# ext-sakamoro/ALICE-Codec

Measured on AMD Instinct MI355X. Metric: Mpixels/s encode+decode, 1080p x 64 CDF9/7 q=80; bit-exact vs CPU, higher is better.
Workload: dtype int32

## Files before the change

alice-codec_amd/csrc/codec.hip:

```cpp
#include <hip/hip_runtime.h>
#include <sys/mman.h>

#include <algorithm>
#include <atomic>
#include <chrono>
#include <condition_variable>
#include <cmath>
#include <cstdio>
#include <cstdlib>
#include <cstring>
#include <exception>
#include <map>
#include <memory>
#include <mutex>
#include <new>
#include <string>
#include <thread>
#include <vector>

#include "../../include/alice_codec.h"
#include "../../include/alice_codec_test.h"
#include "common.h"
#include "kernels.h"

// ... 859 lines not shown
                                 w.hist.as<uint32_t>() + (size_t)b * 3 * 256, w.results.as<RansResult>() + 3 * b,
                                 w.sizes.as<unsigned long long>() + b, 1, st);
    launch_compact_streams(w.alc.as<uint8_t>(), w.alc_stride, kStreamHead, w.cap, w.results.as<RansResult>(), B, st);
    if (evs) HIP_TRY(hipEventRecord(evs->ev[4], st));
    HIP_TRY(hipGetLastError());
    return kOk;
}

int encode_flags_error(uint32_t flags) {
    if (flags & kTableDiverges)
        return fail(kReferenceDiverges, "a symbol whose table frequency wrapped to 0 is present: the reference encoder does not terminate on this input");
    if (flags & kRansInternal) return fail(kInternal, "rANS kernel invariant violated");
    return kOk;
}

constexpr int kOverflowed = -1;

int encode_collect(EncodeWork& w, hipStream_t st, std::vector<RansResult>& res) {
    res.resize((size_t)w.n_chunks * 3);
    HIP_TRY(hipMemcpyAsync(res.data(), w.results.p, res.size() * sizeof(RansResult), hipMemcpyDeviceToHost, st));
    HIP_TRY(hipStreamSynchronize(st));
    for (auto& r : res) TRY(encode_flags_error(r.flags));
    if (debug_on())
        for (size_t i = 0; i < res.size(); ++i)
            fprintf(stderr, "[alice] encode chain %zu: %llu bytes, %.1f Mcycles, %.1f ms of 100 MHz ticks => %.2f GHz, xcc %u se %u cu %u simd %u\n", i, res[i].len,
                    res[i].cycles_k * 1024.0 / 1e6, res[i].ticks_k * 1024.0 / 1e5,
                    res[i].ticks_k ? (res[i].cycles_k / (double)res[i].ticks_k) * 0.1 : 0.0,
                    res[i].xcc_id & 15u, (res[i].hw_id >> 13) & 7u, (res[i].hw_id >> 8) & 15u, (res[i].hw_id >> 4) & 3u);
    for (auto& r : res)
        if (r.flags & kRansOverflow) return kOverflowed;
    return kOk;
}

int encode_with_retry(const RgbLayout* rgb, EncodeWork& w, uint8_t quality, int wavelet, hipStream_t st, StageEvents* evs,
                      CapMode mode, HubTicket* hub, std::vector<RansResult>& res, const uint8_t* qualities = nullptr) {
    for (int m = mode; m <= kCapWorst; ++m) {
        TRY(encode_launch(rgb, w, quality, wavelet, st, evs, (CapMode)m, hub, qualities));
        const int rc = encode_collect(w, st, res);
        if (rc != kOverflowed) return rc;
    }
    return fail(kInternal, "rANS output exceeded the worst-case capacity");
}

struct DecodeWork {
    ChunkDims d{};
    int n_chunks = 0;
    DevBuf scratch_own, gen, tmp, sym, hist, tables, descs, results, planes;
    uint8_t* sym_ptr = nullptr;
    DevBuf* scratch = nullptr;
};

int decode_work_alloc(DecodeWork& w, const ChunkDims& d, int n_chunks, uint8_t* sym_ext = nullptr, DevBuf* scratch_ext = nullptr) {
    w.d = d; w.n_chunks = n_chunks;
    w.scratch = scratch_ext ? scratch_ext : &w.scratch_own;
    if (sym_ext) w.sym_ptr = sym_ext;
    else { TRY(w.sym.alloc((size_t)n_chunks * 3 * d.padded)); w.sym_ptr = w.sym.as<uint8_t>(); }
    TRY(w.hist.alloc((size_t)n_chunks * 3 * 256 * sizeof(uint32_t)));
    TRY(w.tables.alloc((size_t)n_chunks * 3 * sizeof(RansTable)));
    TRY(w.descs.alloc((size_t)n_chunks * 3 * sizeof(RansDecodeDesc)));
    TRY(w.results.alloc((size_t)n_chunks * 3 * sizeof(RansResult)));
    return kOk;
}

int inverse_chunk(const uint8_t* d_sym, const ChunkDims& d, int wavelet, const int32_t step[3], void* d_scratch, DecodeWork& w,
                  const RgbLayout& rgb, hipStream_t st, SplitFormat fmt = kFormatSplit) {
    const bool wide = is_wide(fmt), mirror = fmt == kFormatReversible;
    const InverseBounds ib = inverse_bounds(wavelet, step, wide ? kWideMaxQ : kByteMaxQ);
    if (mirror) {
        if (d_scratch && launch_inverse_transform_reversible((const uint16_t*)d_sym, d, wavelet, step, ib.exact, ib.mid16, ib.lds16, d_scratch, rgb, st))
            return kOk;
    } else if (wide) {
        if (d_scratch && launch_inverse_transform_wide((const uint16_t*)d_sym, d, wavelet, step, ib.exact, ib.mid16, ib.lds16, d_scratch, rgb, st))
            return kOk;
    } else if (d_scratch && launch_inverse_transform(d_sym, d, wavelet, step, ib.exact, ib.mid16, ib.lds16, d_scratch, rgb, st)) return kOk;
    if (!w.planes.p) TRY(w.planes.alloc(3 * d.n_pixels * sizeof(int16_t)));
    if (!w.tmp.p) TRY(w.tmp.alloc(d.padded * sizeof(int32_t)));
    if (!w.gen.p) TRY(w.gen.alloc(2 * d.padded * sizeof(int32_t)));
    int16_t* pl = w.planes.as<int16_t>();
    int32_t* qb = w.gen.as<int32_t>();
    int32_t* vol = qb + d.padded;
    const uint64_t W = d.pw, H = d.ph, D = d.pf;
    for (int c = 0; c < 3; ++c) {
        if (wide) launch_from_symbols_wide((const uint16_t*)d_sym + (size_t)c * d.padded, qb, d.padded, st);
        else launch_from_symbols(d_sym + (size_t)c * d.padded, qb, d.padded, st);
        launch_dequantize(qb, vol, d.padded, step[c], st);
        launch_wavelet_axis(vol, w.tmp.as<int32_t>(), D, W * H, 1, 0, W * H, 1, wavelet, true, st, mirror);
        launch_wavelet_axis(vol, w.tmp.as<int32_t>(), H, W, D, W * H, W, 1, wavelet, true, st, mirror);
        launch_wavelet_axis(vol, w.tmp.as<int32_t>(), W, 1, D * H, W, 1, 0, wavelet, true, st, mirror);
        launch_strip_channel(vol, d, pl + (size_t)c * d.n_pixels, st);
    }
    launch_ycocg_to_rgb(pl, pl + d.n_pixels, pl + 2 * d.n_pixels, d, rgb, st);
    return kOk;
}

int decode_launch(const EncodedChunk* const* headers, const std::vector<const uint8_t*>& d_payload,
                  DecodeWork& w, const std::vector<RgbLayout>& rgb, hipStream_t st, StageEvents* evs, HubTicket* hub = nullptr) {
    const ChunkDims& d = w.d;
    const int B = w.n_chunks;
    if (transform_tiles_eligible(d)) {
        bool all16 = true;
        for (int b = 0; b < B; ++b) {
            const int32_t step[3] = {headers[b]->ch[0].quant_step, headers[b]->ch[1].quant_step, headers[b]->ch[2].quant_step};
            all16 = all16 && inverse_bounds(headers[b]->wavelet, step).mid16;
        }
        const size_t need = inverse_scratch_bytes(d, all16);
        if (!w.scratch->p || w.scratch->n < need) {
            HIP_TRY(hipStreamSynchronize(st));
            TRY(w.scratch->alloc(need));
        }
    }
    std::vector<uint32_t> hist((size_t)B * 3 * 256);
    std::vector<RansDecodeDesc> descs((size_t)B * 3);
    for (int b = 0; b < B; ++b) {
        uint64_t off = 0;
        for (int c = 0; c < 3; ++c) {
            const ChannelHeader& h = headers[b]->ch[c];
            memcpy(&hist[((size_t)b * 3 + c) * 256], h.histogram, 256 * sizeof(uint32_t));
            RansDecodeDesc& ds = descs[(size_t)b * 3 + c];
            ds.in = d_payload[b] + off;
            ds.in_len = h.compressed_len;
            ds.out = w.sym_ptr + ((size_t)b * 3 + c) * d.padded;
            ds.n = d.padded;
            ds.table = w.tables.as<RansTable>() + ((size_t)b * 3 + c);
            off += h.compressed_len;
        }
    }
    HIP_TRY(hipMemcpyAsync(w.hist.p, hist.data(), hist.size() * sizeof(uint32_t), hipMemcpyHostToDevice, st));
    if (!hub) HIP_TRY(hipMemcpyAsync(w.descs.p, descs.data(), descs.size() * sizeof(RansDecodeDesc), hipMemcpyHostToDevice, st));
    HIP_TRY(hipStreamSynchronize(st));
    if (evs) HIP_TRY(hipEventRecord(evs->ev[5], st));
    launch_rans_table(w.hist.as<uint32_t>(), w.tables.as<RansTable>(), 3 * B, st);
    if (hub) {
        for (size_t c = 0; c < descs.size(); ++c) descs[c].result = w.results.as<RansResult>() + c;
        TRY(hub_chains(st, {}, std::move(descs), d.padded, hub));
    } else {
        launch_rans_decode(w.descs.as<RansDecodeDesc>(), w.results.as<RansResult>(), 3 * B, st);
    }
    if (evs) HIP_TRY(hipEventRecord(evs->ev[6], st));
    for (int b = 0; b < B; ++b) {
        const int32_t step[3] = {headers[b]->ch[0].quant_step, headers[b]->ch[1].quant_step, headers[b]->ch[2].quant_step};
        TRY(inverse_chunk(w.sym_ptr + (size_t)b * 3 * d.padded, d, headers[b]->wavelet, step, w.scratch->p, w, rgb[b], st));
    }
    if (evs) HIP_TRY(hipEventRecord(evs->ev[7], st));
    HIP_TRY(hipGetLastError());
    return kOk;
}

int decode_collect(DecodeWork& w, hipStream_t st) {
    std::vector<RansResult> res((size_t)w.n_chunks * 3);
    HIP_TRY(hipMemcpyAsync(res.data(), w.results.p, res.size() * sizeof(RansResult), hipMemcpyDeviceToHost, st));
    HIP_TRY(hipStreamSynchronize(st));
    for (auto& r : res)
        if (r.flags & kRansInternal) return fail(kInternal, "rANS decode table invariant violated");
    if (debug_on())
        for (size_t i = 0; i < res.size(); ++i)
            fprintf(stderr, "[alice] decode chain %zu: consumed %llu bytes, fast tiles %u, slow tiles %u, %.1f Mcycles, xcc %u se %u cu %u simd %u\n", i, res[i].len,
                    res[i].fast_tiles, res[i].slow_tiles, res[i].cycles_k * 1024.0 / 1e6,
                    res[i].xcc_id & 15u, (res[i].hw_id >> 13) & 7u, (res[i].hw_id >> 8) & 15u, (res[i].hw_id >> 4) & 3u);
    return kOk;
}

int validate_for_decode(const EncodedChunk& c, ChunkDims* dims, uint64_t payload_len) {
    uint64_t n_pixels = 0;
    TRY(checked_pixel_count(c.width, c.height, c.frames, &n_pixels));
    *dims = make_dims(c.width, c.height, c.frames);
    if (n_pixels == 0) return kOk;
    uint64_t off = 0;
    for (int k = 0; k < 3; ++k) {
        if ((uint64_t)c.ch[k].num_symbols != dims->padded)
            return fail(kInvalidBitstream, "channel " + std::to_string(k) + ": num_symbols " + std::to_string(c.ch[k].num_symbols) +
                                               " != padded_pixels " + std::to_string(dims->padded));
        if (off + c.ch[k].compressed_len > payload_len)
            return fail(kInvalidBitstream, "channel " + std::to_string(k) + ": compressed data overrun");
        off += c.ch[k].compressed_len;
    }
    return kOk;
}

uint32_t chunks_that_fit(const ChunkDims& d, uint32_t want) {
    if (want <= 1) return want;
    size_t free_b = 0, total_b = 0;
    if (hipMemGetInfo(&free_b, &total_b) != hipSuccess) { (void)hipGetLastError(); return want; }
    const long double per_chunk = (long double)d.n_pixels * 3 + (long double)d.padded * 3 * 2 + 3.0L * sizeof(RansTable) * 2 + 65536;
    const long double fixed = (long double)std::max(forward_scratch_bytes(d), inverse_scratch_bytes(d, false)) + (64u << 20);
    const long double room = (long double)free_b * 0.8L - fixed;
    if (room < per_chunk) return 1;
    const long double n = room / per_chunk;
    return n >= (long double)want ? want : (uint32_t)n;
}

template <typename Slot>
int chunks_to_host(EncodeWork& w, const std::vector<RansResult>& res, hipStream_t st, Slot slot) {
    const uint32_t B = (uint32_t)w.n_chunks;
    std::vector<uint8_t> hdr((size_t)B * kAlcHeaderBytes);
    if (hipMemcpy2DAsync(hdr.data(), kAlcHeaderBytes, w.alc.p, w.alc_stride, kAlcHeaderBytes, B, hipMemcpyDeviceToHost, st) != hipSuccess ||
        hipStreamSynchronize(st) != hipSuccess)
        return fail(kDeviceError, "device to host copy failed");
    return parallel_chunks(B, w.alc_stride >= (4u << 20) ? kCopyThreads : 1u, [&](uint32_t i) {
        const uint64_t payload = res[3 * i].len + res[3 * i + 1].len + res[3 * i + 2].len;
        EncodedChunk* c = slot(i) = new (std::nothrow) EncodedChunk();
        if (!c) return fail(kOutOfMemory, "out of host memory");
        uint64_t tot = 0;
        if (parse_alc_header(hdr.data() + (size_t)i * kAlcHeaderBytes, kAlcHeaderBytes + payload, *c, &tot) != kOk || tot != payload)
            return fail(kInternal, "device header/payload length mismatch");
        c->data.resize((size_t)payload);
        return copy_to_host(c->data.data(), w.alc.as<uint8_t>() + (size_t)i * w.alc_stride + kAlcHeaderBytes, (size_t)payload, st);
    });
}

int check_quality_range(uint8_t min_q, uint8_t max_q) {
    if (std::min<uint8_t>(min_q, 100) > std::min<uint8_t>(max_q, 100)) return fail(kInvalidDimensions, "min_quality > max_quality");
    return kOk;
}

int encode_chunks_on_device(const FrameEncoder& enc, const uint8_t* rgb, const ChunkDims& d, EncodedChunk** out, uint32_t n_chunks,
                            uint32_t slot = 0, uint32_t step = 1) {
    const uint32_t n = slot < n_chunks ? (n_chunks - slot + step - 1) / step : 0;
    auto at = [&](uint32_t i) { return slot + (size_t)i * step; };
    for (uint32_t i = 0; i < n; ++i) out[at(i)] = nullptr;
    if (!n) return kOk;
    TRY(ensure_device());
    const uint32_t per_pass = chunks_that_fit(d, n);
    HubTicket ticket;
    TRY(ticket.open(encode_device_bytes(d, per_pass)));
    const hipStream_t st = ticket.st;
    auto undo = [&](int rc) { for (uint32_t i = 0; i < n; ++i) { delete out[at(i)]; out[at(i)] = nullptr; } return rc; };
    const uint64_t chunk_bytes = d.n_pixels * 3;
    for (uint32_t first = 0; first < n; first += per_pass) {
        const uint32_t B = std::min(per_pass, n - first);
        DevBuf d_rgb;
        EncodeWork w;
        std::vector<RansResult> res;
        int rc = d_rgb.alloc(chunk_bytes * B);
        if (rc == kOk) rc = encode_work_alloc(w, d, (int)B);
        if (rc == kOk)
            rc = parallel_chunks(B, chunk_bytes >= (4u << 20) ? kCopyThreads : 1u, [&](uint32_t i) {
                HIP_TRY(hipMemcpyAsync(d_rgb.as<uint8_t>() + (size_t)i * chunk_bytes, rgb + at(first + i) * chunk_bytes, chunk_bytes, hipMemcpyHostToDevice, st));
                return (int)kOk;
            });
        std::vector<RgbLayout> layouts(B);
        for (uint32_t i = 0; i < B; ++i) layouts[i] = packed_rgb(d_rgb.as<uint8_t>() + (size_t)i * chunk_bytes, d);
        if (rc == kOk) rc = encode_with_retry(layouts.data(), w, enc.quality, enc.wavelet, st, nullptr, kCapReuse, &ticket, res);
        if (rc == kOk) rc = chunks_to_host(w, res, st, [&](uint32_t i) -> EncodedChunk*& { return out[at(first + i)]; });
        if (rc != kOk) return undo(rc);
    }
    return kOk;
}

int decode_chunks_on_device(const EncodedChunk* const* chunks, const ChunkDims& d, uint8_t* rgb_out, uint32_t n_chunks,
                            uint32_t slot = 0, uint32_t step = 1) {
    const uint32_t n = slot < n_chunks ? (n_chunks - slot + step - 1) / step : 0;
    auto at = [&](uint32_t i) { return slot + (size_t)i * step; };
    if (!n || d.n_pixels == 0) return kOk;
    TRY(ensure_device());
    const uint32_t per_pass = chunks_that_fit(d, n);
    uint64_t max_payload = 0;
    for (uint32_t i = 0; i < n; ++i) max_payload = std::max<uint64_t>(max_payload, chunks[at(i)]->data.size());
    HubTicket ticket;
    TRY(ticket.open(decode_device_bytes(d, per_pass, (uint64_t)per_pass * (max_payload + 512))));
    const hipStream_t st = ticket.st;
    const uint64_t chunk_bytes = d.n_pixels * 3;
    for (uint32_t first = 0; first < n; first += per_pass) {
        const uint32_t B = std::min(per_pass, n - first);
        std::vector<const EncodedChunk*> hdrs(B);
        uint64_t total_payload = 0;
        for (uint32_t i = 0; i < B; ++i) { hdrs[i] = chunks[at(first + i)]; total_payload += round_up(hdrs[i]->data.size() + 16, 256); }
        DevBuf d_payload, d_rgb;
        TRY(d_payload.alloc(total_payload + 256));
        TRY(d_rgb.alloc(chunk_bytes * B));
        std::vector<const uint8_t*> pay(B);
        std::vector<RgbLayout> dst(B);
        uint64_t off = 0;
        for (uint32_t i = 0; i < B; ++i) {
            const EncodedChunk& c = *hdrs[i];
            pay[i] = d_payload.as<uint8_t>() + off;
            dst[i] = packed_rgb(d_rgb.as<uint8_t>() + (size_t)i * chunk_bytes, d);
            if (!c.data.empty())
                HIP_TRY(hipMemcpyAsync(d_payload.as<uint8_t>() + off, c.data.data(), c.data.size(), hipMemcpyHostToDevice, st));
            off += round_up(c.data.size() + 16, 256);
        }
        DecodeWork w;
        TRY(decode_work_alloc(w, d, (int)B));
        TRY(decode_launch(hdrs.data(), pay, w, dst, st, nullptr, &ticket));
        TRY(decode_collect(w, st));
        TRY(parallel_chunks(B, chunk_bytes >= (4u << 20) ? kCopyThreads : 1u,
                            [&](uint32_t i) { return copy_to_host(rgb_out + at(first + i) * chunk_bytes, dst[i].base, chunk_bytes, st); }));
    }
    return kOk;
}

int validate_encode_many(const FrameEncoder* encoder, const uint8_t* rgb, uint64_t rgb_len, uint32_t width, uint32_t height,
                         uint32_t frames, uint32_t n_chunks, EncodedChunk** out_chunks, ChunkDims* d) {
    if (!encoder || !out_chunks || (!rgb && rgb_len)) return fail(kNullArgument, "null argument");
    for (uint32_t i = 0; i < n_chunks; ++i) out_chunks[i] = nullptr;
    if (n_chunks == 0) return kOk;
    uint64_t n_pixels = 0;
    TRY(checked_pixel_count(width, height, frames, &n_pixels));
    if (n_pixels == 0 || width == 0 || height == 0) return fail(kInvalidDimensions, "invalid dimensions");
    if (n_pixels > UINT64_MAX / 3 / n_chunks) return fail(kDimensionOverflow, "dimensions overflow usize");
    if (rgb_len != n_pixels * 3 * n_chunks)
        return fail(kInvalidBufferSize, "buffer size mismatch: expected " + std::to_string(n_pixels * 3 * n_chunks) + ", got " + std::to_string(rgb_len));
    return chunk_dims(width, height, frames, d);
}

int encode_host(const FrameEncoder& enc, const uint8_t* rgb, uint64_t rgb_len, uint32_t width, uint32_t height,
                uint32_t frames, EncodedChunk** out) {
// ... 3199 lines not shown
```

alice-codec_amd/csrc/rans.hip:

```cpp
#include <cstdlib>

#include "common.h"
#include "freq_table.h"
#include "kernels.h"

namespace alice {


__device__ inline RansEncEntry make_enc_entry(uint32_t f, uint32_t c) {
    RansEncEntry e;
    e.freq = f;
    e.cum = c;
    unsigned long long xm = (unsigned long long)f << 19;
    unsigned long long xm8 = (unsigned long long)f << 27;
    e.xmax = xm > 0xFFFFFFFFull ? 0xFFFFFFFFu : (uint32_t)xm;
    e.xmax8 = xm8 > 0xFFFFFFFFull ? 0xFFFFFFFFu : (uint32_t)xm8;
    if (f == 0u || f > kProbScale) {
        e.xmax = f == 0u ? 0xFFFFFFFFu : e.xmax;
        e.xmax8 = f == 0u ? 0xFFFFFFFFu : e.xmax8;
        e.rcp = 0u; e.rsh = 0u; e.g = 0; e.cbias = 0u;
    } else if (f == 1u) {
        e.rcp = 0xFFFFFFFFu; e.rsh = 0u; e.g = 4095; e.cbias = c + 4095u;
    } else {
        uint32_t L = 32u - (uint32_t)__clz((int)(f - 1u));
// ... 295 lines not shown
                    asm volatile("" : "+v"(cc_prev));
                    const uint32_t kc = tm1 - cc_prev;
                    uint32_t u = tm1 - xin, z;
                    ripple64_comp(u, z, kc, tpp, rcp, rsh, g);
                    const bool c1 = (int32_t)u < 0;
                    const unsigned long long b1 = __ballot(c1);
                    const uint32_t off = __builtin_amdgcn_mbcnt_hi((uint32_t)(b1 >> 32), __builtin_amdgcn_mbcnt_lo((uint32_t)b1, tw));
                    tb[c1 ? kTileSpan - 1u - off : (uint32_t)lane] = (uint8_t)(~u & 0xFFu);
                    tw += (uint32_t)__popcll(b1);
                    xin = (uint32_t)__builtin_amdgcn_update_dpp(0, (int)(cc - z), 0x13C, 0xf, 0xf, true);
                } else {
                    rare_blocks += 1u;
                    const uint32_t cbias = curp.eb.z, xmax8 = curp.eb.w;
                    uint32_t xout = 0u;
                    const uint32_t cprev = (uint32_t)__builtin_amdgcn_update_dpp(0, (int)cbias, 0x138, 0xf, 0xf, true);
                    const uint32_t k0 = small_f ? 8u : 0u;
                    ripple64_clean(xin, xout, small_f ? xmax8 : xmax, k0, k0 + 8u, rcp, rsh, g, cprev);
                    const bool c1 = xin >= xmax;
                    const bool c2 = xin >= xmax8;
                    const unsigned long long b1 = __ballot(c1), b2 = __ballot(c2);
                    const uint32_t off = __builtin_amdgcn_mbcnt_hi((uint32_t)(b1 >> 32), __builtin_amdgcn_mbcnt_lo((uint32_t)b1, tw)) +
                                         __builtin_amdgcn_mbcnt_hi((uint32_t)(b2 >> 32), __builtin_amdgcn_mbcnt_lo((uint32_t)b2, 0u));
                    tb[c1 ? kTileSpan - 1u - off : (uint32_t)lane] = (uint8_t)(xin & 0xFFu);
                    tb[c2 ? kTileSpan - 2u - off : (uint32_t)lane] = (uint8_t)((xin >> 8) & 0xFFu);
                    tw += (uint32_t)__popcll(b1) + (uint32_t)__popcll(b2);
                    xin = (uint32_t)__builtin_amdgcn_update_dpp(0, (int)(xout + cbias), 0x13C, 0xf, 0xf, false);
                }
                asm volatile("" : "+v"(tw));
            }
            written += (unsigned long long)(uint32_t)__builtin_amdgcn_readfirstlane((int)tw);
            comp_blocks += (uint32_t)(kEncTile / 64) - rare_blocks;
            x = (uint32_t)__builtin_amdgcn_readlane((int)xin, 0);
            continue;
        }
        slow_tiles += 1u;
        paths |= valid < kEncTile ? kEncPathTail : (table_clean ? kEncPathCapRefused : kEncPathNotClean);
        for (int b = 0; b < nblocks; ++b) {
            const BlockParams curp = nxt;
            nxt = params_of(sym1);
            sym1 = sym_of(b + 2);
            const bool active = (kEncTile - 1 - (b * 64 + lane)) >= kEncTile - valid;
            uint4 ea = curp.ea;
            uint4 eb = curp.eb;
            uint2 ec = curp.ec;
            if (!active) {
                ea = make_uint4(0xFFFFFFFFu, 0u, 0u, 0u);
                eb = make_uint4(0u, 0u, 0u, 0xFFFFFFFFu);
                ec = make_uint2(1u, 0u);
            }
            const uint32_t xmax = ea.x, xmax8 = eb.w, rcp = ea.y, rsh = ea.z;
            const int32_t g = (int32_t)ea.w;
            const uint32_t cbias = eb.z, freq = ec.x, cum = ec.y;
            const bool bad = (freq - 1u) >= kProbScale;

            uint32_t xin = x, xout = 0u;
            if (__builtin_expect(__ballot(bad) == 0ull, 1)) {
                uint32_t cprev = (uint32_t)__builtin_amdgcn_update_dpp(0, (int)cbias, 0x138, 0xf, 0xf, true);
                ripple64(xin, xout, xmax, xmax8, rcp, rsh, g, cprev);
                x = (uint32_t)__builtin_amdgcn_readlane((int)xout, 63) +
                    (uint32_t)__builtin_amdgcn_readlane((int)cbias, 63);
            } else {
                paths |= kEncPathExact;
                uint32_t xs = x;
                for (int i = 0; i < 64; ++i) {
                    if (lane == i) xin = xs;
                    const uint32_t fi = (uint32_t)__builtin_amdgcn_readlane((int)freq, i);
                    const uint32_t ci = (uint32_t)__builtin_amdgcn_readlane((int)cum, i);
                    const uint32_t ai = (uint32_t)__builtin_amdgcn_readlane((int)active, i);
                    if (!ai) continue;
                    if (fi == 0u) { flags |= kTableDiverges; continue; }
                    const unsigned long long xm = (unsigned long long)fi << 19;
                    uint32_t ys = xs;
                    while ((unsigned long long)ys >= xm) ys >>= 8;
                    const uint32_t qs = ys / fi, rs = ys % fi;
                    xs = (qs << kProbBits) + rs + ci;
                }
                x = xs;
            }

            const bool c1 = xin >= xmax;
            const bool c2 = xin >= xmax8;
            const unsigned long long b1 = __ballot(c1), b2 = __ballot(c2);
            const uint32_t off = __builtin_amdgcn_mbcnt_hi((uint32_t)(b1 >> 32), __builtin_amdgcn_mbcnt_lo((uint32_t)b1, 0u)) +
                                 __builtin_amdgcn_mbcnt_hi((uint32_t)(b2 >> 32), __builtin_amdgcn_mbcnt_lo((uint32_t)b2, 0u));
            const uint32_t total = (uint32_t)__popcll(b1) + (uint32_t)__popcll(b2);
            const bool room = written + total + 4ull + 64ull <= cap;
            flags |= room ? 0u : kRansOverflow;
            paths |= room ? 0u : kEncPathNoRoom;
            uint8_t* p = out_end - 1 - (written + off);
            uint8_t* p0 = (c1 && room) ? p : dummy;
            uint8_t* p1 = (c2 && room) ? p - 1 : dummy;
            *p0 = (uint8_t)(xin & 0xFFu);
            *p1 = (uint8_t)((xin >> 8) & 0xFFu);
            written += total;
        }
    }

    if (!keep_open) {
        if (written + 4ull + 64ull <= cap) {
            if (lane < 4) out_end[-1 - (long long)(written + lane)] = (uint8_t)((x >> (8 * lane)) & 0xFFu);
        } else {
            flags |= kRansOverflow;
            paths |= kEncPathNoRoom;
        }
        written += 4ull;
    }
    for (uint32_t bit = kEncPathFunnel; bit <= kEncPathBytewiseHead; bit <<= 1)
        paths |= __ballot((load_paths & bit) != 0u) ? bit : 0u;
    const uint32_t clean_tiles = (uint32_t)ntiles - slow_tiles;
    paths |= clean_tiles ? kEncPathClean : 0u;
    if (lane == 0) {
        res->len = written;
        res->flags = flags;
        res->final_state = x;
        res->fast_tiles = clean_tiles;
        res->slow_tiles = slow_tiles;
        res->paths = paths;
        res->comp_blocks = comp_blocks;
        res->cycles_k = (uint32_t)((clock64() - clk0) >> 10);
        res->ticks_k = (uint32_t)((wall_clock64() - rt0) >> 10);
        res->hw_id = __builtin_amdgcn_s_getreg((31 << 11) | 4);
        res->xcc_id = __builtin_amdgcn_s_getreg((31 << 11) | 20);
    }
}


constexpr int kDecBlocks = 64;
constexpr int kDecTile = kDecBlocks * 64;
constexpr int kDecWinBytes = 33 * 64 * 4;
constexpr int kDecWinLds = kDecWinBytes;

#include "rans_decode_tile.inc"

__device__ __forceinline__ void dec_tile_fast(uint32_t& x, uint32_t& pos, const RansDecSlots* slots, uint32_t lane4,
                                              uint32_t win_addr, uint32_t rec_addr, uint32_t nblk) {
    uint32_t xo, po;
    asm volatile(ALICE_DEC_TILE_ASM
                 : [xo] "=&s"(xo), [po] "=&s"(po), [ra] "+v"(rec_addr)
                 : [xi] "s"(x), [pi] "s"(pos), [nb] "s"(nblk), [tp] "s"(slots), [l4] "v"(lane4), [wa] "v"(win_addr)
                 : ALICE_DEC_TILE_CLOBBERS);
    x = xo;
    pos = po;
}

__device__ __forceinline__ void dec_tile_dry(uint32_t& x, const RansDecSlots* slots, uint32_t lane4, uint32_t rec_addr, uint32_t nblk) {
    uint32_t xo;
    asm volatile(ALICE_DEC_DRY_TILE_ASM
                 : [xo] "=&s"(xo), [ra] "+v"(rec_addr)
                 : [xi] "s"(x), [nb] "s"(nblk), [tp] "s"(slots), [l4] "v"(lane4)
                 : ALICE_DEC_DRY_TILE_CLOBBERS);
    x = xo;
}

template <bool kExclusive>
__global__ __launch_bounds__(64) void rans_decode_kernel(const RansDecodeDesc* __restrict__ descs,
                                                         RansResult* __restrict__ results, uint32_t take_turns) {
    if constexpr (kExclusive) asm volatile("" ::: "a63");
    __shared__ __attribute__((aligned(16))) uint8_t c2s[kProbScale];
    __shared__ uint32_t symtab[256];
    __shared__ __attribute__((aligned(16))) uint8_t win[kDecWinLds];
    __shared__ __attribute__((aligned(16))) uint16_t rec[kDecTile];
    uint8_t* const obuf = (uint8_t*)rec;

    const RansDecodeDesc d = descs[blockIdx.x];
    const int lane = threadIdx.x;
    const RansDecSlots* const slots = &d.table->dec;
    uint32_t flags = 0u;
    const uint32_t tflags = d.table->flags;
    const bool big_freq = (tflags & kTableDecBig) != 0u;
    const bool exact_only = (tflags & kTableDecExact) != 0u;
    for (int i = lane; i < (int)kProbScale / 16; i += 64) ((uint4*)c2s)[i] = ((const uint4*)slots->c2s)[i];
    for (int i = lane; i < 256; i += 64) symtab[i] = slots->symtab[i];
    __syncthreads();
    bool slot0_big = false, one_owner = false;
    if (big_freq) {
        const uint32_t o0 = c2s[0];
        slot0_big = symtab[o0] == kProbScale;
        bool same = true;
        for (int i = lane; i < (int)kProbScale; i += 64) same &= c2s[i] == o0;
        one_owner = __ballot(!same) == 0ull;
    }

    uint32_t x = 0u;
    unsigned long long pos = 0ull;
    const unsigned long long len = d.in_len;
    if (d.resume) {
        x = d.x0; pos = d.pos0;
    } else if (len >= 4ull) {
        x = ((uint32_t)d.in[0] << 24) | ((uint32_t)d.in[1] << 16) | ((uint32_t)d.in[2] << 8) | (uint32_t)d.in[3];
        pos = 4ull;
    }
    bool pending = false;
    const unsigned long long clk0 = clock64(), rt0 = wall_clock64();
    unsigned long long done = 0ull;
    uint32_t n_fast = 0u, n_slow = 0u, paths = 0u;

    while (done < d.n) {
        if (!kExclusive) chain_take_turns(take_turns);
        const unsigned long long remain = d.n - done;
        const uint32_t want = remain < (unsigned long long)kDecTile ? (uint32_t)remain : (uint32_t)kDecTile;
        const bool dry_ok = !exact_only && (!slot0_big || (one_owner && x != 0u));
        if (want == (uint32_t)kDecTile && pos >= len && dry_ok) {
            uint32_t xs = (uint32_t)__builtin_amdgcn_readfirstlane((int)x);
            __syncthreads();
            dec_tile_dry(xs, slots, 4u * lane, (uint32_t)(uintptr_t)rec + 2u * lane, (uint32_t)kDecBlocks);
            x = xs;
            __syncthreads();
            const bool out_al = (((uintptr_t)(d.out + done)) & 3u) == 0u;
            paths |= kDecPathDry | (out_al ? 0u : kDecPathUnaligned);
            for (int i = lane * 4; i < kDecTile; i += 256) {
                const uint2 r4 = *(const uint2*)&rec[i];
                const uint32_t packed = (uint32_t)c2s[r4.x & (kProbScale - 1u)] | ((uint32_t)c2s[(r4.x >> 16) & (kProbScale - 1u)] << 8) |
                                        ((uint32_t)c2s[r4.y & (kProbScale - 1u)] << 16) | ((uint32_t)c2s[(r4.y >> 16) & (kProbScale - 1u)] << 24);
                if (out_al) *(uint32_t*)(d.out + done + i) = packed;
                else for (int b = 0; b < 4; ++b) d.out[done + i + b] = (uint8_t)(packed >> (8 * b));
            }
            done += (unsigned long long)kDecTile;
            ++n_fast;
            continue;
        }
        unsigned long long wbase = pos & ~3ull;
        {
            const unsigned long long mis = (unsigned long long)((uintptr_t)(d.in + pos) & 3u);
            if (pos >= mis) wbase = pos - mis;
        }
        const bool whole = (len - wbase >= (unsigned long long)kDecWinLds) && ((((uintptr_t)(d.in + wbase)) & 3u) == 0u);
        __syncthreads();
        if (whole) {
            const uint32_t* g = (const uint32_t*)(d.in + wbase) + lane;
            uint32_t wv[kDecWinLds / 256];
#pragma unroll
            for (int k = 0; k < kDecWinLds / 256; ++k) wv[k] = g[k * 64];
#pragma unroll
            for (int k = 0; k < kDecWinLds / 256; ++k) ((uint32_t*)win)[k * 64 + lane] = wv[k];
        } else {
            for (int i = lane * 4; i < kDecWinLds; i += 64 * 4) {
                const unsigned long long o = wbase + (unsigned long long)i;
                uint32_t w = 0u;
                for (int b = 0; b < 4; ++b)
                    if (o + (unsigned long long)b < len) w |= (uint32_t)d.in[o + b] << (8 * b);
                *(uint32_t*)(win + i) = w;
            }
        }
        __syncthreads();

        uint32_t got = 0u;
        bool fast = (want == (uint32_t)kDecTile) && pos < len && !exact_only;
        const uint32_t x_save = x;
        const unsigned long long pos_save = pos;
        const bool pending_save = pending;
        if (fast && pending) {
            uint32_t xs = x;
            unsigned long long ps = pos;
            int guard = 0;
            while (xs < kRansL && ps < len && guard < 8) { xs = (xs << 8) | (uint32_t)win[ps - wbase]; ps += 1ull; ++guard; }
            if (xs < kRansL) { fast = false; paths |= kDecPathStillStarved; }
            else { x = xs; pos = ps; pending = false; paths |= kDecPathPendingFed; }
        }
        if (fast && x < kRansL) { fast = false; paths |= kDecPathBelowL; }
        if (fast) {
            uint32_t prel = (uint32_t)(pos - wbase);
            uint32_t xs = (uint32_t)__builtin_amdgcn_readfirstlane((int)x);
            prel = (uint32_t)__builtin_amdgcn_readfirstlane((int)prel);
            dec_tile_fast(xs, prel, slots, 4u * lane, (uint32_t)(uintptr_t)win + 4u * lane,
                          (uint32_t)(uintptr_t)rec + 2u * lane, (uint32_t)kDecBlocks);
            x = xs;
            pos = wbase + prel;
            pending = false;
            __syncthreads();
            if (pos > len) {
                x = x_save; pos = pos_save; pending = pending_save;
                fast = false;
                paths |= kDecPathSpecDropped;
            } else {
                paths |= whole ? kDecPathWhole : kDecPathSpecKept;
            }
        }
        if (fast) {
            const bool out_aligned = (((uintptr_t)(d.out + done)) & 3u) == 0u;
            for (int i = lane * 4; i < kDecTile; i += 256) {
                const uint2 r4 = *(const uint2*)&rec[i];
                const uint32_t packed = (uint32_t)c2s[r4.x & (kProbScale - 1u)] | ((uint32_t)c2s[(r4.x >> 16) & (kProbScale - 1u)] << 8) |
                                        ((uint32_t)c2s[r4.y & (kProbScale - 1u)] << 16) | ((uint32_t)c2s[(r4.y >> 16) & (kProbScale - 1u)] << 24);
                if (out_aligned) *(uint32_t*)(d.out + done + i) = packed;
                else *(uint32_t*)(obuf + i) = packed;
            }
            paths |= out_aligned ? 0u : kDecPathUnaligned;
            got = out_aligned ? 0u : (uint32_t)kDecTile;
            done += out_aligned ? (unsigned long long)kDecTile : 0ull;
            ++n_fast;
        } else {
            ++n_slow;
            paths |= kDecPathExact | (want < (uint32_t)kDecTile ? kDecPathTail : 0u);
            __shared__ uint32_t sh_state, sh_cnt, sh_starved;
            __shared__ unsigned long long sh_pos;
            if (lane == 0) {
                uint32_t j = 0u, xs = x;
                unsigned long long ps = pos;
                bool pend = pending;
                const unsigned long long wend = wbase + (unsigned long long)kDecWinBytes;
                bool starved = false;
                while (j < want) {
                    if (pend) {
                        while (xs < kRansL && ps < len) {
                            if (ps >= wend) { starved = true; break; }
                            xs = (xs << 8) | (uint32_t)win[ps - wbase];
                            ps += 1ull;
                        }
                        if (starved) break;
                    }
                    const uint32_t slot = xs & (kProbScale - 1u);
                    const uint32_t sy = c2s[slot];
                    const uint32_t fc = symtab[sy];
                    xs = (fc & 0xFFFFu) * (xs >> kProbBits) + slot - (fc >> 16);
                    obuf[j] = (uint8_t)sy;
                    pend = true;
                    ++j;
                }
                sh_state = xs; sh_pos = ps; sh_cnt = j; sh_starved = starved ? 1u : 0u;
            }
            __syncthreads();
            x = sh_state; pos = sh_pos; got = sh_cnt;
            paths |= sh_starved ? kDecPathStarved : 0u;
            pending = true;
        }
        __syncthreads();
        for (uint32_t i = lane; i < got; i += 64) d.out[done + i] = obuf[i];
        done += got;
    }
    if (pending) {
        while (x < kRansL && pos < len) { x = (x << 8) | (uint32_t)d.in[pos]; pos += 1ull; }
    }
    if (lane == 0) {
        RansResult* const res = d.result ? d.result : results + blockIdx.x;
        res->len = pos;
        res->flags = flags;
        res->final_state = x;
        res->fast_tiles = n_fast;
        res->slow_tiles = n_slow;
        res->paths = paths;
        res->cycles_k = (uint32_t)((clock64() - clk0) >> 10);
        res->ticks_k = (uint32_t)((wall_clock64() - rt0) >> 10);
        res->hw_id = __builtin_amdgcn_s_getreg((31 << 11) | 4);
        res->xcc_id = __builtin_amdgcn_s_getreg((31 << 11) | 20);
    }
}


void launch_rans_table(const uint32_t* d_hist, RansTable* d_tables, int n_chains, hipStream_t st, uint32_t n_symbols,
                       const uint32_t* d_used) {
    if (n_chains <= 0) return;
    hipLaunchKernelGGL(rans_table_kernel, dim3(n_chains), dim3(256), 0, st, d_hist, d_tables, n_symbols, d_used);
}

void launch_rans_table_from_arrays(const uint16_t* d_cum, const uint16_t* d_freq, RansTable* d_table,
                                   hipStream_t st) {
    hipLaunchKernelGGL(rans_table_from_arrays_kernel, dim3(1), dim3(256), 0, st, d_cum, d_freq, d_table);
}

static uint32_t chain_turns_enabled() {
    static const uint32_t on = [] { const char* v = getenv("ALICE_CHAIN_TURNS"); return (v && *v == '1') ? 1u : 0u; }();
    return on;
}

static unsigned chain_lds_pad(int n_chains, unsigned static_lds) {
    if (n_chains <= 1024 || n_chains > 2048) return 0u;
    const unsigned want = 163840u / 8u - 1024u;
    return want > static_lds ? want - static_lds : 0u;
}

struct ChainKernelFacts { bool ok; unsigned enc_regs, enc_lds, enc_wg_per_cu, dec_regs, dec_lds, dec_wg_per_cu, enc_lds_plain, dec_lds_plain; };
static const ChainKernelFacts& chain_kernel_facts() {
    static const ChainKernelFacts f = [] {
        ChainKernelFacts r{};
        hipFuncAttributes a{};
        int nb = 0;
        r.ok = true;
        auto q = [&](const void* fn, unsigned& regs, unsigned& lds, unsigned* wg) {
            if (hipFuncGetAttributes(&a, fn) != hipSuccess) { r.ok = false; (void)hipGetLastError(); return; }
            regs = (unsigned)a.numRegs; lds = (unsigned)a.sharedSizeBytes;
            if (wg) {
                if (hipOccupancyMaxActiveBlocksPerMultiprocessor(&nb, fn, 64, 0) != hipSuccess) { r.ok = false; (void)hipGetLastError(); return; }
                *wg = (unsigned)nb;
            }
        };
        unsigned dummy = 0;
        q((const void*)rans_encode_kernel<true>, r.enc_regs, r.enc_lds, &r.enc_wg_per_cu);
        q((const void*)rans_decode_kernel<true>, r.dec_regs, r.dec_lds, &r.dec_wg_per_cu);
        q((const void*)rans_encode_kernel<false>, dummy, r.enc_lds_plain, nullptr);
        q((const void*)rans_decode_kernel<false>, dummy, r.dec_lds_plain, nullptr);
        return r;
    }();
    return f;
}
bool chain_kernel_occupancy(uint32_t out[6]) {
    const ChainKernelFacts& f = chain_kernel_facts();
    out[0] = f.enc_regs; out[1] = f.enc_lds; out[2] = f.enc_wg_per_cu;
    out[3] = f.dec_regs; out[4] = f.dec_lds; out[5] = f.dec_wg_per_cu;
    return f.ok;
}

void launch_rans_encode(const uint8_t* d_sym, uint64_t sym_stride, uint64_t n, const RansTable* d_tables,
                        uint8_t* d_out, uint64_t cap, RansResult* d_results, int n_chains, hipStream_t st,
                        uint64_t group_stride, uint64_t group_head, unsigned n_split, uint64_t cap_co, uint64_t cap_cg,
                        uint32_t x_init, bool keep_open) {
    if (n_chains <= 0) return;
    auto kern = n_chains <= 1024 ? rans_encode_kernel<true> : rans_encode_kernel<false>;
    const ChainKernelFacts& facts = chain_kernel_facts();
    hipLaunchKernelGGL(kern, dim3(n_chains), dim3(64), chain_lds_pad(n_chains, facts.ok ? facts.enc_lds_plain : 9216u), st, d_sym,
                       (unsigned long long)sym_stride, (unsigned long long)n, d_tables, d_out,
                       (unsigned long long)cap, (unsigned long long)group_stride, (unsigned long long)group_head, n_split,
                       d_results, (unsigned long long)(cap_co ? cap_co : cap), (unsigned long long)(cap_cg ? cap_cg : cap),
                       x_init, keep_open ? 1u : 0u, chain_turns_enabled(), (const RansEncodeDesc*)nullptr);
}

void launch_rans_encode_descs(const RansEncodeDesc* d_descs, int n_chains, hipStream_t st) {
    if (n_chains <= 0) return;
    auto kern = n_chains <= 1024 ? rans_encode_kernel<true> : rans_encode_kernel<false>;
    const ChainKernelFacts& facts = chain_kernel_facts();
    hipLaunchKernelGGL(kern, dim3(n_chains), dim3(64), chain_lds_pad(n_chains, facts.ok ? facts.enc_lds_plain : 9216u), st,
                       (const uint8_t*)nullptr, 0ull, 0ull, (const RansTable*)nullptr, (uint8_t*)nullptr, 0ull, 0ull, 0ull, 0xFFFFFFFFu,
                       (RansResult*)nullptr, 0ull, 0ull, kRansL, 0u, chain_turns_enabled(), d_descs);
}

void launch_rans_decode(const RansDecodeDesc* d_descs, RansResult* d_results, int n_chains, hipStream_t st) {
    if (n_chains <= 0) return;
    auto kern = n_chains <= 1024 ? rans_decode_kernel<true> : rans_decode_kernel<false>;
    const ChainKernelFacts& facts = chain_kernel_facts();
    hipLaunchKernelGGL(kern, dim3(n_chains), dim3(64), chain_lds_pad(n_chains, facts.ok ? facts.dec_lds_plain : 21776u + 256u), st, d_descs, d_results,
                       chain_turns_enabled());
}

}
```

Measured before the change: 11790.

## Chain consecutive fast rANS decode tiles, prefetching next window during symbol writeback

The fast decode path now loops over consecutive whole tiles. While the current tile's symbols are looked up and written out, it loads the next input window from global memory and stores it into LDS, so each tile no longer goes back through the outer loop setup. Descriptor fields, state and position are forced into scalar registers with readfirstlane to cut VGPR address work. An optional compile-time probe records cycles spent in fast tiles. The change adds scheduling barriers and more complex control flow, with some risk of register pressure.

```diff
diff --git a/alice-codec_amd/csrc/codec.hip b/alice-codec_amd/csrc/codec.hip
--- a/alice-codec_amd/csrc/codec.hip
+++ b/alice-codec_amd/csrc/codec.hip
@@ -1035,6 +1035,12 @@
     HIP_TRY(hipStreamSynchronize(st));
     for (auto& r : res)
         if (r.flags & kRansInternal) return fail(kInternal, "rANS decode table invariant violated");
+#ifdef ALICE_PROBE_DEC_TILE_CYCLES
+    if (debug_on())
+        for (size_t i = 0; i < res.size(); ++i)
+            fprintf(stderr, "[alice] decode probe chain %zu: fast tiles %u, slow tiles %u, total %u Kcycles, in fast tiles %u Kcycles\n", i,
+                    res[i].fast_tiles, res[i].slow_tiles, res[i].cycles_k, res[i].ticks_k);
+#endif
     if (debug_on())
         for (size_t i = 0; i < res.size(); ++i)
             fprintf(stderr, "[alice] decode chain %zu: consumed %llu bytes, fast tiles %u, slow tiles %u, %.1f Mcycles, xcc %u se %u cu %u simd %u\n", i, res[i].len,
diff --git a/alice-codec_amd/csrc/rans.hip b/alice-codec_amd/csrc/rans.hip
--- a/alice-codec_amd/csrc/rans.hip
+++ b/alice-codec_amd/csrc/rans.hip
@@ -471,6 +471,70 @@
     x = xo;
 }
 
+typedef __attribute__((address_space(1))) uint32_t GlobalWord;
+typedef __attribute__((address_space(1))) const uint32_t GlobalConstWord;
+__device__ __forceinline__ uint32_t uniform32(uint32_t v) { return (uint32_t)__builtin_amdgcn_readfirstlane((int)v); }
+__device__ __forceinline__ unsigned long long uniform64(unsigned long long v) {
+    return ((unsigned long long)uniform32((uint32_t)(v >> 32)) << 32) | (unsigned long long)uniform32((uint32_t)v);
+}
+
+__device__ __forceinline__ unsigned long long dec_window_base(const uint8_t* in, unsigned long long pos) {
+    const unsigned long long mis = (unsigned long long)((uintptr_t)(in + pos) & 3u);
+    return pos >= mis ? pos - mis : (pos & ~3ull);
+}
+__device__ __forceinline__ bool dec_window_whole(const uint8_t* in, unsigned long long wbase, unsigned long long len) {
+    return (len - wbase >= (unsigned long long)kDecWinLds) && ((((uintptr_t)(in + wbase)) & 3u) == 0u);
+}
+
+__device__ __forceinline__ void dec_window_load(uint32_t (&wv)[kDecWinLds / 256], const uint8_t* in, unsigned long long wbase, int lane) {
+    GlobalConstWord* const g = (GlobalConstWord*)uniform64((unsigned long long)(uintptr_t)(in + wbase));
+#pragma unroll
+    for (int k = 0; k < kDecWinLds / 256; ++k) wv[k] = g[(uint32_t)(k * 64 + lane)];
+}
+__device__ __forceinline__ void dec_window_store(const uint32_t (&wv)[kDecWinLds / 256], uint8_t* win, int lane) {
+#pragma unroll
+    for (int k = 0; k < kDecWinLds / 256; ++k) ((uint32_t*)win)[k * 64 + lane] = wv[k];
+}
+
+constexpr int kDecSymTrips = kDecTile / 256;
+__device__ __forceinline__ void dec_tile_symbols_read(uint32_t (&packed)[kDecSymTrips], const uint16_t* rec, const uint8_t* c2s, int lane) {
+    uint2 r4[kDecSymTrips];
+#pragma unroll
+    for (int k = 0; k < kDecSymTrips; ++k) r4[k] = *(const uint2*)&rec[k * 256 + lane * 4];
+    uint32_t slot[4 * kDecSymTrips], sy[4 * kDecSymTrips];
+#pragma unroll
+    for (int k = 0; k < kDecSymTrips; ++k) {
+        slot[4 * k + 0] = r4[k].x & (kProbScale - 1u);
+        slot[4 * k + 1] = (r4[k].x >> 16) & (kProbScale - 1u);
+        slot[4 * k + 2] = r4[k].y & (kProbScale - 1u);
+        slot[4 * k + 3] = (r4[k].y >> 16) & (kProbScale - 1u);
+    }
+    __builtin_amdgcn_sched_barrier(0);
+#pragma unroll
+    for (int j = 0; j < 4 * kDecSymTrips; ++j) sy[j] = (uint32_t)c2s[slot[j]];
+    __builtin_amdgcn_sched_barrier(0);
+#pragma unroll
+    for (int k = 0; k < kDecSymTrips; ++k) packed[k] = sy[4 * k] | (sy[4 * k + 1] << 8) | (sy[4 * k + 2] << 16) | (sy[4 * k + 3] << 24);
+}
+__device__ __forceinline__ bool dec_tile_symbols_write(const uint32_t (&packed)[kDecSymTrips], uint8_t* out, uint8_t* obuf, int lane) {
+    const unsigned long long out_u = uniform64((unsigned long long)(uintptr_t)out);
+    const bool out_aligned = (out_u & 3ull) == 0ull;
+    if (__builtin_expect(out_aligned, 1)) {
+        GlobalWord* const g = (GlobalWord*)out_u;
+#pragma unroll
+        for (int k = 0; k < kDecSymTrips; ++k) g[(uint32_t)(k * 64 + lane)] = packed[k];
+    } else {
+#pragma unroll
+        for (int k = 0; k < kDecSymTrips; ++k) ((uint32_t*)obuf)[k * 64 + lane] = packed[k];
+    }
+    return out_aligned;
+}
+__device__ __forceinline__ bool dec_tile_symbols(const uint16_t* rec, const uint8_t* c2s, uint8_t* out, uint8_t* obuf, int lane) {
+    uint32_t packed[kDecSymTrips];
+    dec_tile_symbols_read(packed, rec, c2s, lane);
+    return dec_tile_symbols_write(packed, out, obuf, lane);
+}
+
 template <bool kExclusive>
 __global__ __launch_bounds__(64) void rans_decode_kernel(const RansDecodeDesc* __restrict__ descs,
                                                          RansResult* __restrict__ results, uint32_t take_turns) {
@@ -481,11 +545,15 @@
     __shared__ __attribute__((aligned(16))) uint16_t rec[kDecTile];
     uint8_t* const obuf = (uint8_t*)rec;
 
-    const RansDecodeDesc d = descs[blockIdx.x];
+    RansDecodeDesc d = descs[blockIdx.x];
+    d.in = (const uint8_t*)uniform64((unsigned long long)(uintptr_t)d.in);
+    d.in_len = uniform64(d.in_len);
+    d.out = (uint8_t*)uniform64((unsigned long long)(uintptr_t)d.out);
+    d.n = uniform64(d.n);
     const int lane = threadIdx.x;
     const RansDecSlots* const slots = &d.table->dec;
     uint32_t flags = 0u;
-    const uint32_t tflags = d.table->flags;
+    const uint32_t tflags = uniform32(d.table->flags);
     const bool big_freq = (tflags & kTableDecBig) != 0u;
     const bool exact_only = (tflags & kTableDecExact) != 0u;
     for (int i = lane; i < (int)kProbScale / 16; i += 64) ((uint4*)c2s)[i] = ((const uint4*)slots->c2s)[i];
@@ -509,10 +577,21 @@
         x = ((uint32_t)d.in[0] << 24) | ((uint32_t)d.in[1] << 16) | ((uint32_t)d.in[2] << 8) | (uint32_t)d.in[3];
         pos = 4ull;
     }
+    x = uniform32(x);
+    pos = uniform64(pos);
     bool pending = false;
     const unsigned long long clk0 = clock64(), rt0 = wall_clock64();
     unsigned long long done = 0ull;
     uint32_t n_fast = 0u, n_slow = 0u, paths = 0u;
+#ifdef ALICE_PROBE_DEC_TILE_CYCLES
+    unsigned long long tile_clk = 0ull;
+#endif
+
+    auto flush_obuf = [&](uint32_t cnt) {
+        __syncthreads();
+        for (uint32_t i = lane; i < cnt; i += 64) d.out[done + i] = obuf[i];
+        __syncthreads();
+    };
 
     while (done < d.n) {
         if (!kExclusive) chain_take_turns(take_turns);
@@ -525,33 +604,20 @@
             dec_tile_dry(xs, slots, 4u * lane, (uint32_t)(uintptr_t)rec + 2u * lane, (uint32_t)kDecBlocks);
             x = xs;
             __syncthreads();
-            const bool out_al = (((uintptr_t)(d.out + done)) & 3u) == 0u;
+            const bool out_al = dec_tile_symbols(rec, c2s, d.out + done, obuf, lane);
             paths |= kDecPathDry | (out_al ? 0u : kDecPathUnaligned);
-            for (int i = lane * 4; i < kDecTile; i += 256) {
-                const uint2 r4 = *(const uint2*)&rec[i];
-                const uint32_t packed = (uint32_t)c2s[r4.x & (kProbScale - 1u)] | ((uint32_t)c2s[(r4.x >> 16) & (kProbScale - 1u)] << 8) |
-                                        ((uint32_t)c2s[r4.y & (kProbScale - 1u)] << 16) | ((uint32_t)c2s[(r4.y >> 16) & (kProbScale - 1u)] << 24);
-                if (out_al) *(uint32_t*)(d.out + done + i) = packed;
-                else for (int b = 0; b < 4; ++b) d.out[done + i + b] = (uint8_t)(packed >> (8 * b));
-            }
+            if (!out_al) flush_obuf((uint32_t)kDecTile);
             done += (unsigned long long)kDecTile;
             ++n_fast;
             continue;
         }
-        unsigned long long wbase = pos & ~3ull;
-        {
-            const unsigned long long mis = (unsigned long long)((uintptr_t)(d.in + pos) & 3u);
-            if (pos >= mis) wbase = pos - mis;
-        }
-        const bool whole = (len - wbase >= (unsigned long long)kDecWinLds) && ((((uintptr_t)(d.in + wbase)) & 3u) == 0u);
+        unsigned long long wbase = dec_window_base(d.in, pos);
+        bool whole = dec_window_whole(d.in, wbase, len);
         __syncthreads();
         if (whole) {
-            const uint32_t* g = (const uint32_t*)(d.in + wbase) + lane;
             uint32_t wv[kDecWinLds / 256];
-#pragma unroll
-            for (int k = 0; k < kDecWinLds / 256; ++k) wv[k] = g[k * 64];
-#pragma unroll
-            for (int k = 0; k < kDecWinLds / 256; ++k) ((uint32_t*)win)[k * 64 + lane] = wv[k];
+            dec_window_load(wv, d.in, wbase, lane);
+            dec_window_store(wv, win, lane);
         } else {
             for (int i = lane * 4; i < kDecWinLds; i += 64 * 4) {
                 const unsigned long long o = wbase + (unsigned long long)i;
@@ -565,24 +631,30 @@
 
         uint32_t got = 0u;
         bool fast = (want == (uint32_t)kDecTile) && pos < len && !exact_only;
-        const uint32_t x_save = x;
-        const unsigned long long pos_save = pos;
-        const bool pending_save = pending;
+        uint32_t x_save = x;
+        unsigned long long pos_save = pos;
+        bool pending_save = pending;
         if (fast && pending) {
             uint32_t xs = x;
             unsigned long long ps = pos;
             int guard = 0;
             while (xs < kRansL && ps < len && guard < 8) { xs = (xs << 8) | (uint32_t)win[ps - wbase]; ps += 1ull; ++guard; }
+            xs = uniform32(xs);
             if (xs < kRansL) { fast = false; paths |= kDecPathStillStarved; }
-            else { x = xs; pos = ps; pending = false; paths |= kDecPathPendingFed; }
+            else { x = xs; pos = uniform64(ps); pending = false; paths |= kDecPathPendingFed; }
         }
         if (fast && x < kRansL) { fast = false; paths |= kDecPathBelowL; }
-        if (fast) {
-            uint32_t prel = (uint32_t)(pos - wbase);
-            uint32_t xs = (uint32_t)__builtin_amdgcn_readfirstlane((int)x);
-            prel = (uint32_t)__builtin_amdgcn_readfirstlane((int)prel);
+        while (fast) {
+            uint32_t prel = uniform32((uint32_t)(pos - wbase));
+            uint32_t xs = uniform32(x);
+#ifdef ALICE_PROBE_DEC_TILE_CYCLES
+            const unsigned long long tclk0 = clock64();
+#endif
             dec_tile_fast(xs, prel, slots, 4u * lane, (uint32_t)(uintptr_t)win + 4u * lane,
                           (uint32_t)(uintptr_t)rec + 2u * lane, (uint32_t)kDecBlocks);
+#ifdef ALICE_PROBE_DEC_TILE_CYCLES
+            tile_clk += clock64() - tclk0;
+#endif
             x = xs;
             pos = wbase + prel;
             pending = false;
@@ -591,19 +663,31 @@
                 x = x_save; pos = pos_save; pending = pending_save;
                 fast = false;
                 paths |= kDecPathSpecDropped;
-            } else {
-                paths |= whole ? kDecPathWhole : kDecPathSpecKept;
+                break;
             }
+            paths |= whole ? kDecPathWhole : kDecPathSpecKept;
+            const unsigned long long nbase = dec_window_base(d.in, pos);
+            const bool again = d.n - done >= 2ull * (unsigned long long)kDecTile && x >= kRansL && dec_window_whole(d.in, nbase, len);
+            if (!again) break;
+            if (!kExclusive) chain_take_turns(take_turns);
+            uint32_t wv[kDecWinLds / 256];
+            dec_window_load(wv, d.in, nbase, lane);
+            uint32_t packed[kDecSymTrips];
+            dec_tile_symbols_read(packed, rec, c2s, lane);
+            __builtin_amdgcn_sched_barrier(0);
+            dec_window_store(wv, win, lane);
+            __builtin_amdgcn_sched_barrier(0);
+            const bool out_al = dec_tile_symbols_write(packed, d.out + done, obuf, lane);
+            paths |= out_al ? 0u : kDecPathUnaligned;
+            if (!out_al) flush_obuf((uint32_t)kDecTile);
+            done += (unsigned long long)kDecTile;
+            ++n_fast;
+            __syncthreads();
+            wbase = nbase; whole = true;
+            x_save = x; pos_save = pos; pending_save = false;
         }
         if (fast) {
-            const bool out_aligned = (((uintptr_t)(d.out + done)) & 3u) == 0u;
-            for (int i = lane * 4; i < kDecTile; i += 256) {
-                const uint2 r4 = *(const uint2*)&rec[i];
-                const uint32_t packed = (uint32_t)c2s[r4.x & (kProbScale - 1u)] | ((uint32_t)c2s[(r4.x >> 16) & (kProbScale - 1u)] << 8) |
-                                        ((uint32_t)c2s[r4.y & (kProbScale - 1u)] << 16) | ((uint32_t)c2s[(r4.y >> 16) & (kProbScale - 1u)] << 24);
-                if (out_aligned) *(uint32_t*)(d.out + done + i) = packed;
-                else *(uint32_t*)(obuf + i) = packed;
-            }
+            const bool out_aligned = dec_tile_symbols(rec, c2s, d.out + done, obuf, lane);
             paths |= out_aligned ? 0u : kDecPathUnaligned;
             got = out_aligned ? 0u : (uint32_t)kDecTile;
             done += out_aligned ? (unsigned long long)kDecTile : 0ull;
@@ -639,12 +723,11 @@
                 sh_state = xs; sh_pos = ps; sh_cnt = j; sh_starved = starved ? 1u : 0u;
             }
             __syncthreads();
-            x = sh_state; pos = sh_pos; got = sh_cnt;
-            paths |= sh_starved ? kDecPathStarved : 0u;
+            x = uniform32(sh_state); pos = uniform64(sh_pos); got = uniform32(sh_cnt);
+            paths |= uniform32(sh_starved) ? kDecPathStarved : 0u;
             pending = true;
         }
-        __syncthreads();
-        for (uint32_t i = lane; i < got; i += 64) d.out[done + i] = obuf[i];
+        flush_obuf(got);
         done += got;
     }
     if (pending) {
@@ -659,7 +742,12 @@
         res->slow_tiles = n_slow;
         res->paths = paths;
         res->cycles_k = (uint32_t)((clock64() - clk0) >> 10);
+#ifdef ALICE_PROBE_DEC_TILE_CYCLES
+        res->ticks_k = (uint32_t)(tile_clk >> 10);
+        (void)rt0;
+#else
         res->ticks_k = (uint32_t)((wall_clock64() - rt0) >> 10);
+#endif
         res->hw_id = __builtin_amdgcn_s_getreg((31 << 11) | 4);
         res->xcc_id = __builtin_amdgcn_s_getreg((31 << 11) | 20);
     }
```

After: 11900, median of 6. Within noise of the previous version (+0.9%).
